# huangnengCSU/longcallR

Hardware: AMD Instinct MI355X
Metric: candidate_sites_per_sec (higher is better)
Workload: dtype u8 in, u32 counts, f64 likelihoods, i64 fixed-point phase scores

## Files before the change

### longcallr_amd/api.py

```python
import ctypes as C

import numpy as np

from . import _abi, _lib
from ._lib import LcrError


def _view(ptr, dtype, n):
    if n == 0 or not ptr:
        return np.zeros(0, dtype=dtype)
    buf = (C.c_char * (np.dtype(dtype).itemsize * n)).from_address(ptr)
    return np.frombuffer(buf, dtype=dtype, count=n).copy()


def _view_nocopy(ptr, dtype, n):
    if n == 0 or not ptr:
        return np.zeros(0, dtype=dtype)
    buf = (C.c_char * (np.dtype(dtype).itemsize * n)).from_address(ptr)
    return np.frombuffer(buf, dtype=dtype, count=n)


_DEBUG_ENV = {"LCR_PHASE_PROF": "phase_prof", "LCR_GRID_MIN_ENTRIES": "grid_min_entries",
              "LCR_GRID_GENERIC": "grid_generic", "LCR_GRID_SPEC_LANES": "grid_spec_lanes", "LCR_GRID_SPEC_BATCH": "grid_spec_batch", "LCR_POST_HALF": "post_half", "LCR_ENUM_FORCE_BIG": "enum_force_big",
              "LCR_ENUM_FORCE_STREAM": "enum_force_stream", "LCR_HIST_TILES": "hist_tiles", "LCR_TIE_ARITH": "tie_arith", "LCR_CHAIN_TIES": "chain_ties", "LCR_K3_HITS": "k3_hits", "LCR_FUSE_FILTER": "fuse_filter", "LCR_ASYNC_PHASE": "async_phase", "LCR_HOST_TRACE": "host_trace", "LCR_OWN_FILL": "own_fill", "LCR_REDO_LDS": "redo_lds", "LCR_SPEC_COMPACT": "spec_compact"}


class Engine:
    def __init__(self, device=0, params=None, timing=False):
        self.lib = _lib.load()
        h = C.c_void_p()
        rc = self.lib.lcr_ctx_create(device, C.byref(h))
        if rc != 0:
            raise LcrError("lcr_ctx_create(device=%d) failed with %d: no usable HIP device; "
                           "liblcr has no CPU fallback" % (device, rc))
        self.h = h
        self.device = device
        self.params = params if params is not None else _abi.make_params()
        self._sites = None
        self._keep = None
        self.last_truncated_columns = 0
        if timing:
            self.lib.lcr_enable_timing(self.h, 1)
            if timing is not True:
                self.debug_set("timing_mask", sum(1 << int(k) for k in timing))
        import os
        for env, key in _DEBUG_ENV.items():
            v = os.environ.get(env)
# ... 242 lines not shown
```

### longcallr_amd/csrc/k1_pileup.hip

```cpp
#include <algorithm>
#include <climits>

#include "lcr_dev.h"
#include "k2_eval.h"

#ifdef LCR_K1_ABLATE
#define K1_ABL LCR_K1_ABLATE
#else
#define K1_ABL 0
#endif
#ifndef K1_THREADS
#define K1_THREADS LCR_TILE
#endif
#define K1_WAVES (K1_THREADS / 64)
#define K1_CPT (LCR_TILE / K1_THREADS)
#define K1_RPB 2
#define K1_PMAP (8 * K1_THREADS)
#ifndef K1_NT_STORES
#define K1_NT_STORES 0
#endif
#ifndef K1_PIF
#define K1_PIF 4
#endif

// ... 165 lines not shown
  P_DIFF_DEPTH_R,
  P_DIFF_TS0,
  P_DIFF_TS1,
  P_DIFF_D,
  P_DIFF_N,
  P_NI,
  P_MM_F,
  P_MM_R = P_MM_F + 4,
  P_NPL = P_MM_R + 4
};
#define TSTRIDE (LCR_TILE + 1)
#define REF_PAD 16

__device__ __forceinline__ int block_incl_scan(int v, int* wsum ) {
  const int lane = threadIdx.x & 63, w = threadIdx.x >> 6;
  int s = wave_incl_scan(v);
  if (lane == 63) wsum[w] = s;
  __syncthreads();
  int add = 0;
  for (int i = 0; i < w; i++) add += wsum[i];
  return s + add;
}

__global__ void __launch_bounds__(K1_THREADS)
k1_pileup(BatchView b, DevParams prm, const int32_t* __restrict__ tile_region, const int32_t* __restrict__ tile_col0,
          int64_t n_cols, const int32_t* __restrict__ tile_fill, const int32_t* __restrict__ ent_off, const uint2* __restrict__ ents,
          const unsigned long long* __restrict__ recs,
          const int32_t* __restrict__ tile_nbase, uint32_t* __restrict__ planes, const int32_t* __restrict__ order,
          const int32_t* __restrict__ n_full, BinomTable bt, uint8_t* __restrict__ flt_flags, int32_t* __restrict__ flt_count) {
  if ((int)blockIdx.x >= *n_full) return;
  const int tile = order[blockIdx.x];
  __shared__ uint32_t pl[P_NPL * TSTRIDE];
  __shared__ __attribute__((aligned(16))) uint8_t refl[REF_PAD + LCR_TILE + 32];
  __shared__ unsigned long long rec_s[K1_RPB * K1_THREADS];
  __shared__ int pstart[K1_RPB * K1_THREADS + 1];
  __shared__ uint16_t pown[K1_PMAP];
  __shared__ int wsum[K1_WAVES];

  const int tid = threadIdx.x;
  const int g = tile_region[tile];
  const int tc0 = tile_col0[tile];
  const int vec = b.len[g];
  const int tlen = min(LCR_TILE, vec - tc0);
  const int64_t gcol0 = b.col_off[g] + tc0;
  if (*b.error_flag != 0) return;
  __shared__ uint32_t vge[17], vlt[17];
// ... 176 lines not shown
    __syncthreads();
  }

  const uint32_t nbase = (uint32_t)tile_nbase[tile];
  static_assert(K1_CPT == 1, "the fused filter counts one column per thread");
  int n_pass = 0;
  for (int col = tid; col < tlen; col += K1_THREADS) {
    const uint8_t R = refl[REF_PAD + col];
    const int ri = R == 'A' ? 0 : R == 'C' ? 1 : R == 'G' ? 2 : R == 'T' ? 3 : -1;
    uint32_t f[4], rv[4];
    uint32_t sf = 0, sr = 0;
#pragma unroll
    for (int k = 0; k < 4; k++) {
      const int hk = k < 2 ? k : 5 - k;
      f[k] = pl[(P_MM_F + hk) * TSTRIDE + col]; rv[k] = pl[(P_MM_R + hk) * TSTRIDE + col];
      sf += f[k]; sr += rv[k];
    }
    if (ri >= 0) {
      const uint32_t mf = pl[P_DIFF_DEPTH_F * TSTRIDE + col] - sf, mr = pl[P_DIFF_DEPTH_R * TSTRIDE + col] - sr;
#pragma unroll
      for (int k = 0; k < 4; k++) if (k == ri) { f[k] = mf; rv[k] = mr; }
    }
    const int64_t o = gcol0 + col;
#pragma unroll
    for (int k = 0; k < 4; k++) {
      planes[(int64_t)(LCR_PL_A + k) * n_cols + o] = f[k] + rv[k];
      planes[(int64_t)(LCR_PL_FWD_A + k) * n_cols + o] = f[k];
    }
    planes[(int64_t)LCR_PL_N * n_cols + o] = nbase + pl[P_DIFF_N * TSTRIDE + col];
    planes[(int64_t)LCR_PL_D * n_cols + o] = pl[P_DIFF_D * TSTRIDE + col];
    planes[(int64_t)LCR_PL_NI * n_cols + o] = pl[P_NI * TSTRIDE + col];
    planes[(int64_t)LCR_PL_TS_FWD * n_cols + o] = pl[P_DIFF_TS0 * TSTRIDE + col];
    planes[(int64_t)LCR_PL_TS_REV * n_cols + o] = pl[P_DIFF_TS1 * TSTRIDE + col];
    if (flt_flags) {
      uint32_t cnt[4];
#pragma unroll
      for (int k = 0; k < 4; k++) cnt[k] = f[k] + rv[k];
      const ColEval ev = eval_counts(cnt, R, prm, bt, [&]() { return pl[P_DIFF_D * TSTRIDE + col]; }, [&]() { return nbase + pl[P_DIFF_N * TSTRIDE + col]; },
                                     [&](int k) { return f[k]; });
      flt_flags[o] = ev.pass ? 1 : 0;
      n_pass += ev.pass ? 1 : 0;
    }
  }
  if (flt_flags) {
    const int total = __syncthreads_count(n_pass);
    if (tid == 0) flt_count[tile] = total;
  }
}

__global__ void __launch_bounds__(128) k1_empty_tiles(BatchView b, const int32_t* __restrict__ tile_region, const int32_t* __restrict__ tile_col0,
                                                       int64_t n_cols, const int32_t* __restrict__ tile_nbase, uint32_t* __restrict__ planes,
                                                       const int32_t* __restrict__ order, const int32_t* __restrict__ n_full, int n_tiles) {
  const int nf = *n_full;
  if (*b.error_flag != 0) return;
  const int bt = blockIdx.x, lt = threadIdx.x;
  if (bt + nf >= n_tiles) return;
  const int tile = order[nf + bt];
  const int g = tile_region[tile], tc0 = tile_col0[tile];
  const int tlen = min(LCR_TILE, b.len[g] - tc0);
  const int64_t gcol0 = b.col_off[g] + tc0;
  const uint32_t nb = (uint32_t)tile_nbase[tile];
  for (int col = lt * 4; col < tlen; col += 128 * 4) {
// ... 120 lines not shown
  for (int i = 0; i < w; i++) { run_d += ws[i][0]; run_c += ws[i][1]; }
  int e_before = ie - my_e;
  for (int i = 0; i < w; i++) e_before += we[i];
  if (tid < 33) hist[tid] = 0;
  __syncthreads();
#pragma unroll
  for (int x = 0; x < 4; x++) {
    const int t = t0 + x;
    if (t < n_tiles) {
      run_d += vd[x]; tile_nbase[t] = run_d;
      ent_off[t] = run_c; run_c += vc[x];
      if (cls[x] == 32) {
        order[base[32] + e_before++] = t;
        if (flt_count) flt_count[t] = 0;
      } else order[base[cls[x]] + atomicAdd(&hist[cls[x]], 1)] = t;
      if (t == n_tiles - 1) { ent_off[n_tiles] = run_c; tmp->n_full = n_tiles - tmp->cls_cnt[32]; }
    }
  }
}

void launch_k1_pileup(const BatchView& b, const DevParams& p, const int32_t* tile_region, const int32_t* tile_col0,
                      int32_t n_tiles, int64_t n_cols, const int32_t* tile_fill, const int32_t* ent_off, const void* ents,
                      const unsigned long long* recs, const int32_t* tile_nbase, uint32_t* planes, const int32_t* order ,
                      const int32_t* tiles_tmp, hipStream_t s, uint8_t* flt_flags, int32_t* flt_count) {
  static const BinomTable bt = make_binom_table();
  if (n_tiles == 0) return;
  hipLaunchKernelGGL(k1_pileup, dim3(n_tiles), dim3(K1_THREADS), 0, s, b, p, tile_region, tile_col0, n_cols, tile_fill, ent_off,
                     (const uint2*)ents, recs, tile_nbase, planes, order, tiles_tmp + 80 , bt, flt_flags, flt_count);
}
void launch_k1_empty_tiles(const BatchView& b, const int32_t* tile_region, const int32_t* tile_col0, int32_t n_tiles, int64_t n_cols,
                           const int32_t* tile_nbase, uint32_t* planes, const int32_t* order, const int32_t* tiles_tmp, hipStream_t s) {
  if (n_tiles == 0) return;
  hipLaunchKernelGGL(k1_empty_tiles, dim3(n_tiles), dim3(128), 0, s, b, tile_region, tile_col0, n_cols, tile_nbase, planes, order, tiles_tmp + 80, n_tiles);
}
size_t launch_k1_tiles_tmp_words(int32_t n_tiles) { return 88 + 2 * (size_t)((n_tiles + TS_TILES - 1) / TS_TILES) + 8; }
void launch_k1_tiles_a(int32_t n_tiles, const int32_t* tile_fill, const int32_t* tile_ndiff, const int32_t* tile_nent, int32_t* tmp ,
                       const unsigned int* acct, int32_t n_acct, K0Ctl* ctl, K0Ctl* host_ctl, const int32_t* tile_region,
                       const int32_t* tile_col0, const int32_t* region_len, hipStream_t s) {
  const int nb = (n_tiles + TS_TILES - 1) / TS_TILES;
  hipLaunchKernelGGL(k1_tiles_a, dim3(nb), dim3(256), 0, s, tile_fill, tile_ndiff, tile_nent, n_tiles, (TileScanTmp*)tmp, (int2*)(tmp + 88), acct, n_acct, ctl, host_ctl,
                     tile_region, tile_col0, region_len);
}
void launch_k1_tiles_b(int32_t n_tiles, const int32_t* tile_fill, const int32_t* tile_ndiff, const int32_t* tile_nent, int32_t* tmp,
                       int32_t* tile_nbase, int32_t* ent_off, int32_t* order, int32_t* flt_count, hipStream_t s) {
  const int nb = (n_tiles + TS_TILES - 1) / TS_TILES;
  hipLaunchKernelGGL(k1_tiles_b, dim3(nb), dim3(256), 0, s, tile_fill, tile_ndiff, tile_nent, n_tiles, (TileScanTmp*)tmp, (const int2*)(tmp + 88),
                     tile_nbase, ent_off, order, flt_count);
}

__global__ void __launch_bounds__(LCR_BLOCK)
k1_zonefix(BatchView b, int D, int L, int64_t n_cols, uint32_t* __restrict__ planes) {
// ... 234 lines not shown
```

### longcallr_amd/csrc/lcr_api.hip

```cpp
#include <chrono>
#include <cmath>
#include <cstdlib>
#include <map>
#include <mutex>

#include "lcr_ctx.h"

namespace {
struct BlockCache {
  std::mutex mu;
  std::multimap<size_t, void*> blocks[2][16];
  size_t held[2][16] = {};
  size_t limit[2] = {(size_t)24 << 30, (size_t)2 << 30};
};
BlockCache& block_cache() { static BlockCache* c = new BlockCache(); return *c; }
}
void* lcr_cache_take(int host, size_t want, size_t* cap) {
  int dev = 0;
  if (hipGetDevice(&dev) != hipSuccess || dev < 0 || dev >= 16) return nullptr;
  BlockCache& bc = block_cache();
  std::lock_guard<std::mutex> g(bc.mu);
  auto& m = bc.blocks[host ? 1 : 0][dev];
  auto it = m.lower_bound(want);
  if (it == m.end() || it->first > 2 * want + (1u << 20)) return nullptr;
// ... 440 lines not shown
        uint8_t* base = buf.as<uint8_t>();
        HIPCHK(c, lcr_fill_async(base + off, 0x5C, len, c->stream));
        std::fill(want.begin() + off, want.begin() + off + len, (uint8_t)0x5C);
        void* const ptrs[4] = {base + N + off, base + 2 * N + 3, nullptr, base + 3 * N + off};
        const int vals[4] = {0x80, 0, 7, 0xFF};
        const size_t sizes[4] = {len, 33, 0, len / 2};
        HIPCHK(c, lcr_fill_multi_async(4, ptrs, vals, sizes, c->stream));
        std::fill(want.begin() + N + off, want.begin() + N + off + len, (uint8_t)0x80);
        std::fill(want.begin() + 2 * N + 3, want.begin() + 2 * N + 3 + 33, (uint8_t)0);
        std::fill(want.begin() + 3 * N + off, want.begin() + 3 * N + off + len / 2, (uint8_t)0xFF);
        HIPCHK(c, hipMemcpyAsync(host.data(), buf.p, 4 * N, hipMemcpyDeviceToHost, c->stream));
        HIPCHK(c, hipStreamSynchronize(c->stream));
        if (host != want) { c->err = "fill_selftest: a fill kernel wrote other bytes than asked (offset " + std::to_string(off) + ", length " + std::to_string(len) + ")"; return LCR_E_DEVICE; }
      }
  }
  else if (k == "chain_ties") d.chain_ties = value != 0;
  else if (k == "redo_lds") d.redo_lds = (int)std::max<int64_t>(0, std::min<int64_t>(value, 128 * 1024));
  else if (k == "tie_arith") d.tie_arith = (int)std::max<int64_t>(0, std::min<int64_t>(value, 3));
  else if (k == "timing_mask") c->timing_mask = (uint32_t)value;
  else if (k == "hist_tiles") c->dbg_hist_tiles = value > 0 ? 1 : value < 0 ? -1 : 0;
  else if (k == "k3_hits") c->dbg_k3_hits = value != 0;
  else if (k == "fuse_filter") c->dbg_fuse_filter = value != 0;
  else if (k == "spec_compact") c->dbg_spec_compact = value != 0;
  else if (k == "poison_planes") c->dbg_poison_planes = value != 0;
  else if (k == "grid_spec_batch") d.spec_batch = (int)value;
  else if (k == "grid_spec_lanes") d.spec_lanes = (int)std::max<int64_t>(1, std::min<int64_t>(value, 16));
  else { c->err = "lcr_debug_set: unknown key " + k; return LCR_E_ARG; }
  return LCR_OK;
}

int lcr_get_ld_blocks(lcr_ctx* c, int32_t region, int32_t* n_blocks, const int32_t** block_off, const int32_t** snp_idx) {
  if (!c || !n_blocks || !block_off || !snp_idx) return LCR_E_ARG;
  if (c->stage < ST_PHASED) { c->err = "lcr_get_ld_blocks before lcr_phase"; return LCR_E_STATE; }
  if (region < 0 || region >= c->bv.n_regions) { c->err = "lcr_get_ld_blocks: no such region"; return LCR_E_ARG; }
  { int rc = phase_settle(c); if (rc) return rc; }
  PhaseInputs in;
  in.n_regions = c->bv.n_regions;
  in.cand_region_off = c->h_cand_off.data();
  const int rc = c->phase.ld_blocks(in, region, &c->ld_off, &c->ld_snps, c->stream, &c->err);
  if (rc != LCR_OK) return rc;
  *n_blocks = (int32_t)c->ld_off.size() - 1; *block_off = c->ld_off.data(); *snp_idx = c->ld_snps.data();
  return LCR_OK;
}

int lcr_get_tie_census(lcr_ctx* c, uint64_t out[8]) {
  if (!c || !out) return LCR_E_ARG;
// ... 8 lines not shown
```

### longcallr_amd/csrc/lcr_calls.hip

```cpp
#include "lcr_ctx.h"

int cand_settle(lcr_ctx* c) {
  if (!c->cand_pending) return LCR_OK;
  HIPCHK(c, hipEventSynchronize(c->ev_cand));
  const int ng = c->bv.n_regions;
  memcpy(c->h_cand_off.data(), c->h_stage[2].p, (size_t)(ng + 1) * 4);
  c->h_cand.assign(c->h_stage[1].as<lcr_candidate>(), c->h_stage[1].as<lcr_candidate>() + c->h_cand_off[ng]);
  c->cand_pending = false;
  return LCR_OK;
}

int frag_settle(lcr_ctx* c) {
  if (!c->nnz_pending) return LCR_OK;
  HIPCHK(c, hipEventSynchronize(c->ev_nnz));
  c->nnz = c->h_nnz.as<int64_t>()[c->bv.n_regions];
  c->nnz_pending = false;
  return LCR_OK;
}

namespace {

void cand_begin(lcr_ctx* c) {
  c->res_valid = false;
  rewind_to(c, ST_PILED);
// ... 13 lines not shown
  c->stage = ST_CALLED;
  return LCR_OK;
}

int cand_host_blocks(lcr_ctx* c, size_t n_max, lcr_candidate** hp, int32_t** ho) {
  const int ng = c->bv.n_regions;
  HIPCHK(c, c->h_stage[1].reserve(std::max<size_t>(n_max, 1) * sizeof(lcr_candidate)));
  HIPCHK(c, c->h_stage[2].reserve((size_t)(ng + 1) * 4));
  HIPCHK(c, c->h_stage[1].dev(hp));
  HIPCHK(c, c->h_stage[2].dev(ho));
  if (ng == 0) c->h_stage[2].as<int32_t>()[0] = 0;
  return LCR_OK;
}

int cand_queue_pass1(lcr_ctx* c) {
  const int nt = c->n_tiles;
  HIPCHK(c, c->flags.reserve(std::max<size_t>(c->n_cols, 1)));
  HIPCHK(c, c->tile_count.reserve(std::max(nt, 1) * 4));
  HIPCHK(c, c->tile_off.reserve((std::max(nt, 1) + 1) * 4));
  HIPCHK(c, c->total.reserve(16));
  const DevParams &fa = c->flt_dp, &fb = c->dp;
  const bool have_flt = c->flt_fused && c->dbg_fuse_filter != 0 && fa.ont == fb.ont && fa.min_depth == fb.min_depth && fa.max_depth == fb.max_depth && fa.low_cnt_cut == fb.low_cnt_cut &&
                        fa.use_strand_bias == fb.use_strand_bias && fa.min_af_intron == fb.min_af_intron && fa.low_frac_cut == fb.low_frac_cut && fa.sor_threshold == fb.sor_threshold;
  Timer t(c, LCR_K_CAND_FILTER);
  if (!have_flt) {
    c->flt_fused = false;
    launch_k2_filter(c->bv, c->dp, c->tile_region.as<int32_t>(), c->tile_col0.as<int32_t>(), nt, c->n_cols,
                     c->planes.as<uint32_t>(), c->k0_tile_fill.as<int32_t>(), c->flags.as<uint8_t>(), c->tile_count.as<int32_t>(), c->stream);
  }
  return LCR_OK;
}

void queue_compact(lcr_ctx* c, int32_t cap) {
  launch_k2_compact(c->bv, c->dp, c->tile_region.as<int32_t>(), c->tile_col0.as<int32_t>(), c->n_tiles, c->n_cols,
                    c->planes.as<uint32_t>(), c->flags.as<uint8_t>(), c->tile_count.as<int32_t>(), c->tile_off.as<int32_t>(),
                    c->survivors.as<Survivor>(), cap, c->stream);
}

int cand_count_survivors(lcr_ctx* c, int32_t* n_sv_out, bool* compacted) {
  const int ng = c->bv.n_regions, nt = c->n_tiles;
  HIPCHK(c, c->sv_region_off.reserve((ng + 1) * 4));
  HIPCHK(c, c->h_stage[0].reserve((ng + 2) * 4));
  int32_t* const sv_off = c->h_stage[0].as<int32_t>();
  { int32_t* d_sv = nullptr;
    HIPCHK(c, c->h_stage[0].dev(&d_sv));
    launch_scan_i32(c->scan_tmp, c->tile_count.as<int32_t>(), c->tile_off.as<int32_t>(), nt, c->total.as<int32_t>(), c->stream);
// ... 116 lines not shown
  const int64_t* d_pos = nullptr; const uint8_t* d_gt = nullptr; const float* d_q = nullptr;
  { int rc = upload(c, c->imp_pos, pos0, (size_t)n_sites, &d_pos, mem); if (rc) return rc; }
  { int rc = upload(c, c->imp_gt, genotype, (size_t)n_sites, &d_gt, mem); if (rc) return rc; }
  { int rc = upload(c, c->imp_q, qual, (size_t)n_sites, &d_q, mem); if (rc) return rc; }
  if (mem == LCR_MEM_DEVICE && n_sites > 0) {
    HIPCHK(c, c->h_imp_bad.reserve(64));
    int32_t* bad = c->h_imp_bad.as<int32_t>();
    *bad = 0;
    int32_t* d_bad = nullptr;
    HIPCHK(c, c->h_imp_bad.dev(&d_bad));
    launch_k2_import_check(d_pos, d_gt, n_sites, d_bad, c->stream);
    HIPCHK(c, hipEventRecord(c->ev_imp, c->stream));
    HIPCHK(c, hipEventSynchronize(c->ev_imp));
    if (*(volatile int32_t*)bad) { c->err = "lcr_import_candidates: sites must be sorted by position without duplicates, genotype codes 0-4"; return LCR_E_ARG; }
  }
  cand_begin(c);
  HIPCHK(c, c->imp_cnt.reserve(std::max(ng, 1) * 4));
  HIPCHK(c, c->d_cand.reserve(std::max<size_t>(n_sites, 1) * sizeof(lcr_candidate)));
  HIPCHK(c, c->d_cand_off.reserve((ng + 1) * 4));
  lcr_candidate* hp = nullptr; int32_t* ho = nullptr;
  { int rc = cand_host_blocks(c, (size_t)n_sites, &hp, &ho); if (rc) return rc; }
  c->h_cand.clear();
  c->h_cand_off.assign(ng + 1, 0);
  { Timer t(c, LCR_K_CAND_IMPORT);
    launch_k2_import_count(c->bv, d_pos, d_gt, d_q, n_sites, c->imp_cnt.as<int32_t>(), c->stream);
    launch_scan_i32(c->scan_tmp, c->imp_cnt.as<int32_t>(), c->d_cand_off.as<int32_t>(), ng, c->d_cand_off.as<int32_t>() + ng, c->stream);
    launch_k2_import_emit(c->bv, c->n_cols, c->planes.as<uint32_t>(), c->k0_tile_fill.as<int32_t>(), d_pos, d_gt, d_q, n_sites, c->d_cand_off.as<int32_t>(),
                          c->d_cand.as<lcr_candidate>(), c->stream, hp, ho); }
  const int rc = cand_tail(c);
  HT("import:ret");
  return rc;
}

int lcr_get_candidates(lcr_ctx* c, lcr_candidate_list* out) {
  if (!c || !out) return LCR_E_ARG;
  if (c->stage < ST_CALLED) { c->err = "lcr_get_candidates before lcr_candidates"; return LCR_E_STATE; }
  { int rc = cand_settle(c); if (rc) return rc; }
  { int rc = phase_settle(c); if (rc) return rc; }
  out->n_cand = (int32_t)c->h_cand.size();
  out->n_regions = c->bv.n_regions;
  out->cand = c->h_cand.data();
  out->region_off = c->h_cand_off.data();
  return LCR_OK;
}

int lcr_get_candidates_device(lcr_ctx* c, const lcr_candidate** dev_cand, int32_t* n_cand) {
// ... 111 lines not shown
```

### longcallr_amd/csrc/lcr_ctx.h

```cpp
#pragma once
#include <algorithm>
#include <cstring>

#include "lcr_dev.h"
#include "lcr_phase_host.h"

enum Stage { ST_NONE, ST_LOADED, ST_PILED, ST_CALLED, ST_FRAGGED, ST_PHASED };

struct lcr_ctx {
  int device = 0;
  hipStream_t stream = nullptr;
  bool own_stream = false;
  std::string err;
  Stage stage = ST_NONE;

  BatchView bv{};
  int64_t n_cols = 0, n_bases = 0, n_cigar = 0;
  int32_t n_tiles = 0;
  std::vector<int64_t> h_start0, h_col_off;
  std::vector<int32_t> h_len, h_read_begin, h_region_first_tile;
  DevBuf in_[16];
  struct UploadSlot { DevBuf buf[16]; hipEvent_t ev = nullptr; bool filled = false; lcr_reads rd{}; lcr_regions rg{}; } up[2];
  hipStream_t up_stream = nullptr;
  int bound_slot = -1;
  bool bound_host = false;
  DevBuf scan_tmp, read_region, read_bin, read_rend, tile_region, tile_col0, first_tile, k0_tile_fill, k0_items, tile_nbase, tile_order;
  DevBuf desc_tile, desc_val, chunks, chunk_off;
  DevBuf blk_first_read, read_scan, cig_compact, cig_off_new, cig_new_off32;
  uint64_t cig0 = 0;
  uint32_t n_ops = 0;
  int64_t n_items = 0;

  bool planes_dense = false;
  int dbg_poison_planes = 0;
  DevBuf planes;
  DevParams dp{};
  int32_t pile_platform = -1; uint32_t pile_dist_to_end = 0;
  float sor_thr = -1.f;
  HostBuf h_planes;
  HostBuf h_nnz;
  DevBuf region_e_off, frag_tmp_col, frag_tmp_val;
  hipEvent_t ev_ctl = nullptr, ev_sv = nullptr, ev_cand = nullptr, ev_nnz = nullptr, ev_imp = nullptr;
  int32_t sv_cap_guess = 0;
  bool nnz_pending = false, cand_pending = false;
  HostBuf h_order;
  static constexpr int UP_LANES = 4;
  HostBuf h_up[2 * UP_LANES]; hipEvent_t ev_up[2 * UP_LANES] = {}; bool up_busy[2 * UP_LANES] = {};
  HostBuf h_stage[4];

  bool cand_used = false;
  DevBuf flags, tile_count, tile_off, total, survivors, sv_region_off, hist, cand_tmp, keep;
  DevBuf hit_cnt, hit_list, ovf_list;
  bool hits_valid = false; int32_t hits_n_sv = 0;
  int dbg_hist_tiles = 0;
  int dbg_spec_compact = 1;
  int dbg_fuse_filter = 1;
// ... 22 lines not shown
  std::vector<uint8_t> ds_rows; bool ds_rows_set = false;

  bool junc_valid = false;
  int32_t junc_n = 0, junc_ng = 0;
  DevBuf j_part, j_npair, j_part_off, j_pair_off, j_tsz, j_tbl_off, j_rows, j_keys, j_tbl_key, j_tbl_cnt, j_flag, j_koff, j_ck, j_cc, j_cg, j_off, d_junc;
  HostBuf h_junc_ctl, h_junc, h_junc_off;
  hipEvent_t ev_junc = nullptr;

  DevBuf rd_start, rd_end, rd_diff, rd_ex, rd_cnt, rd_off, rd_s, rd_e, rd_max;
  std::vector<int64_t> rl_start0;
  std::vector<int32_t> rl_len;
  std::vector<uint32_t> rl_max;

  bool timing = false;
  uint32_t timing_mask = 0;
  hipEvent_t ev[LCR_NKERNELS][2] = {};
  bool ev_valid[LCR_NKERNELS] = {};
  int64_t pileup_bytes = 0, stage_bytes = 0;
};

inline void rewind_to(lcr_ctx* c, Stage to) {
  if (c->stage > to) c->stage = to;
  if (to < ST_PILED) {
    c->planes_dense = false;
    c->flt_fused = false;
  }
  if (to < ST_CALLED) {
    c->hits_valid = false;
    c->cand_used = false;
  }
  if (to < ST_FRAGGED) c->ds_rows_set = false;
  if (to < ST_PHASED) c->junc_valid = false;
}

struct Timer {
  lcr_ctx* c; int k;
  bool on() const { return c->timing && (c->timing_mask == 0 || ((c->timing_mask >> k) & 1u)); }
  Timer(lcr_ctx* c_, int k_) : c(c_), k(k_) { if (on()) { (void)hipEventRecord(c->ev[k][0], c->stream); } }
  ~Timer() { if (on()) { (void)hipEventRecord(c->ev[k][1], c->stream); c->ev_valid[k] = true; } }
};

inline DevParams to_dev(const lcr_params* p, float sor_thr) {
  DevParams d{};
  d.ont = p->platform == LCR_PLATFORM_ONT;
  d.dist_to_end = (int32_t)p->dist_to_end;
  d.polya_len = (int32_t)p->polya_len;
  d.min_baseq = p->min_baseq; d.min_depth = p->min_depth; d.max_depth = p->max_depth; d.min_qual = p->min_qual;
  d.low_cnt_cut = p->low_cnt_cut; d.min_linkers = p->min_linkers; d.use_strand_bias = p->use_strand_bias;
  d.min_af = p->min_af; d.min_af_intron = p->min_af_intron; d.low_frac_cut = p->low_frac_cut;
  d.sor_threshold = sor_thr;
  return d;
}

int upload_bytes(lcr_ctx* c, void* dst, const void* src, size_t bytes, hipStream_t q = nullptr);

template <class T>
int upload(lcr_ctx* c, DevBuf& buf, const T* src, size_t n, const T** dst, int mem) {
  if (mem == LCR_MEM_DEVICE) { *dst = src; return LCR_OK; }
  HIPCHK(c, buf.reserve(std::max<size_t>(n, 1) * sizeof(T)));
  if (n) { const int rc = upload_bytes(c, buf.p, src, n * sizeof(T)); if (rc) return rc; }
  *dst = buf.as<T>();
  return LCR_OK;
}

inline int phase_settle(lcr_ctx* c) { return c->phase.settle(&c->err); }
int cand_settle(lcr_ctx* c);
int frag_settle(lcr_ctx* c);
```

### longcallr_amd/csrc/lcr_dev.h

```cpp
#pragma once
#include <hip/hip_runtime.h>
#include <climits>
#include <cstddef>
#include <stdint.h>

#include <string>
#include <vector>

#include "../../include/lcr.h"

#ifndef LCR_TILE
#define LCR_TILE 256
#endif
#define LCR_BLOCK 256
#define LCR_WAVE 64

struct BatchView {
  int32_t n_reads, n_regions;
  int64_t n_bases;
  const int32_t* pos;
  const int32_t* seq_len;
  const int32_t* lead;
  const int32_t* trail;
  const uint8_t* flags;
// ... 161 lines not shown
  size_t nch;
  size_t cur;
  size_t acct;
  size_t tmp;
  size_t words;
};
inline PileScratch pile_scratch(int32_t n_tiles) {
  const size_t nt = (size_t)n_tiles;
  PileScratch L{};
  L.ctl = nt + 1; L.ndiff = nt + 16; L.nch = L.ndiff + nt + 8; L.cur = L.nch + nt + 8; L.acct = L.cur + nt + 8;
  L.tmp = L.acct + launch_k0_acct_words();
  L.words = (L.tmp + launch_k1_tiles_tmp_words(n_tiles) + 63) & ~(size_t)63;
  return L;
}
void launch_k1_tiles_a(int32_t n_tiles, const int32_t* tile_fill, const int32_t* tile_ndiff, const int32_t* tile_nent, int32_t* tmp ,
                       const unsigned int* acct, int32_t n_acct, K0Ctl* ctl, K0Ctl* host_ctl ,
                       const int32_t* tile_region, const int32_t* tile_col0, const int32_t* region_len , hipStream_t s);
void launch_k1_tiles_b(int32_t n_tiles, const int32_t* tile_fill, const int32_t* tile_ndiff, const int32_t* tile_nent, int32_t* tmp,
                       int32_t* tile_nbase, int32_t* ent_off, int32_t* order, int32_t* flt_count , hipStream_t s);
void launch_k1_pileup(const BatchView& b, const DevParams& p, const int32_t* tile_region, const int32_t* tile_col0,
                      int32_t n_tiles, int64_t n_cols, const int32_t* tile_fill, const int32_t* chunk_off, const void* chunks,
                      const unsigned long long* recs, const int32_t* tile_nbase, uint32_t* planes, const int32_t* order,
                      const int32_t* tiles_tmp , hipStream_t s,
                      uint8_t* flt_flags , int32_t* flt_count );
void launch_k1_empty_tiles(const BatchView& b, const int32_t* tile_region, const int32_t* tile_col0, int32_t n_tiles, int64_t n_cols,
                           const int32_t* tile_nbase, uint32_t* planes, const int32_t* order, const int32_t* tiles_tmp, hipStream_t s);
void launch_k1_zonefix(const BatchView& b, const ReadBin* rbin, int D, int L, int64_t n_cols, uint32_t* planes, hipStream_t s);
void launch_k2_filter(const BatchView& b, const DevParams& p, const int32_t* tile_region, const int32_t* tile_col0,
                      int32_t n_tiles, int64_t n_cols, const uint32_t* planes, const int32_t* tile_fill, uint8_t* flags,
                      int32_t* tile_count, hipStream_t s);
void launch_gather_i32(const int32_t* src, const int32_t* idx, int32_t n, int32_t n_src, const int32_t* total, int32_t* out, hipStream_t s,
                       int32_t* host_out = nullptr );
void launch_scan_i32(DevBuf& tmp, const int32_t* in, int32_t* out_excl, int32_t n, int32_t* total, hipStream_t s);
void launch_k2_compact(const BatchView& b, const DevParams& p, const int32_t* tile_region, const int32_t* tile_col0,
                       int32_t n_tiles, int64_t n_cols, const uint32_t* planes, const uint8_t* flags,
                       const int32_t* tile_count, const int32_t* tile_off, Survivor* out, int32_t out_cap, hipStream_t s);
float lcr_device_sor_threshold(hipStream_t s);
#define LCR_HITS 16
void launch_k2_hist(const BatchView& b, const DevParams& p, const ReadBin* rbin, const Survivor* sv, const int32_t* tile_off , int32_t n_tiles, int32_t n_sv,
                    uint32_t* hist , int32_t* hit_cnt , void* hit_list ,
                    int32_t* ovf_cnt , int32_t* ovf_list , hipStream_t s);
void launch_k2_hist_tiles(const BatchView& b, const int32_t* tile_col0, int32_t n_tiles, const int32_t* tile_count,
                          const int32_t* tile_off, const Survivor* sv, const int32_t* ent_off, const void* ents, const unsigned long long* recs,
                          uint32_t* hist, hipStream_t s);
void launch_k2_gt(const DevParams& p, const Survivor* sv, int32_t n_sv, const uint32_t* hist, const int64_t* start0,
                  lcr_candidate* out, int32_t* keep, hipStream_t s);
void launch_k2_finish(DevBuf& scan_tmp, const lcr_candidate* tmp, const int32_t* keep, int32_t n_sv, const int32_t* sv_region_off,
// ... 188 lines not shown
```

### longcallr_amd/csrc/lcr_pileup.hip

```cpp
#include "lcr_ctx.h"

namespace {

struct PilePools {
  int32_t n_blocks = 0;
  size_t pool_cap64 = 0, desc_cap64 = 0;
  size_t n_shards = 0;
  unsigned int pool_sub = 0, desc_sub = 0;
};

PilePools pile_size_pools(const lcr_ctx* c) {
  PilePools P;
  const int opb = launch_k0_opb();
  P.n_blocks = (int32_t)(((uint64_t)c->n_ops + opb - 1) / opb);
  P.desc_cap64 = (size_t)P.n_blocks * 128 + (size_t)c->bv.n_reads / 4 + 1024;
  P.pool_cap64 = (size_t)c->n_ops + (size_t)c->n_ops / 2 + (size_t)c->bv.n_reads + (size_t)c->n_bases / LCR_TILE + 8 * P.desc_cap64 + 1024;
  return P;
}

int pile_reserve_pools(lcr_ctx* c, PilePools& P) {
  const size_t nsh = P.n_shards = (size_t)launch_k0_acct_slots();
  const size_t pool_sub64 = (P.pool_cap64 + nsh - 1) / nsh + 256, desc_sub64 = (P.desc_cap64 + nsh - 1) / nsh + 64;
  if (pool_sub64 * nsh > 0xFFFFFFF0ull || desc_sub64 * nsh > 0x7FFFFFF0ull) { c->err = "batch too large for the 32-bit record pool: split it"; return LCR_E_ARG; }
  P.pool_sub = (unsigned int)pool_sub64; P.desc_sub = (unsigned int)desc_sub64;
// ... 7 lines not shown
int pile_reserve_scratch(lcr_ctx* c, const PileScratch& L) {
  const int nt = c->n_tiles;
  HIPCHK(c, c->k0_tile_fill.reserve(L.words * 4));
  c->bv.error_flag = &reinterpret_cast<K0Ctl*>(c->k0_tile_fill.as<int32_t>() + L.ctl)->error;
  HIPCHK(c, c->tile_order.reserve(std::max(nt, 1) * 4));
  HIPCHK(c, c->tile_nbase.reserve(std::max(nt, 1) * 4));
  HIPCHK(c, c->chunk_off.reserve(((size_t)nt + 2) * 4));
  HIPCHK(c, c->read_scan.reserve(std::max<size_t>(c->bv.n_reads, 1) * 8));
  HIPCHK(c, c->h_stage[0].reserve(64));
  return LCR_OK;
}

int pile_queue_k0(lcr_ctx* c, const PileScratch& L, const PilePools& P, bool& gated) {
  int32_t* const fill = c->k0_tile_fill.as<int32_t>();
  HIPCHK(c, lcr_fill_async(fill, 0, L.words * 4, c->stream));
  if (!gated) { HIPCHK(c, c->phase.gate_stream(c->stream)); gated = true; }
  Timer t(c, LCR_K_SPANS);
  launch_k0_ops(c->bv, c->read_bin.as<ReadBin>(), c->blk_first_read.as<int32_t>(), c->cig0, c->n_ops, c->dp.ont, c->dp.dist_to_end, c->n_tiles,
                fill, fill + L.nch, fill + L.ndiff, reinterpret_cast<K0Ctl*>(fill + L.ctl), (unsigned int*)(fill + L.acct), P.pool_sub, c->k0_items.as<unsigned long long>(),
                P.desc_sub, c->desc_tile.as<uint32_t>(), c->desc_val.p, c->read_scan.p, c->stream);
  return LCR_OK;
}

int pile_queue_tally(lcr_ctx* c, const PileScratch& L, const PilePools& P, bool fuse) {
  BatchView& b = c->bv;
  const int nt = c->n_tiles;
  int32_t* const fill = c->k0_tile_fill.as<int32_t>();
  K0Ctl* const d_ctl = reinterpret_cast<K0Ctl*>(fill + L.ctl);
  { Timer t(c, LCR_K_PILEUP);
    if (nt > 0) {
      K0Ctl* h_ctl_dev = nullptr;
      HIPCHK(c, c->h_stage[0].dev(&h_ctl_dev));
      launch_k1_tiles_a(nt, fill, fill + L.ndiff, fill + L.nch, fill + L.tmp, (unsigned int*)(fill + L.acct), launch_k0_acct_slots(),
                        d_ctl, h_ctl_dev, c->tile_region.as<int32_t>(), c->tile_col0.as<int32_t>(), b.len, c->stream);
    } else HIPCHK(c, hipMemcpyAsync(c->h_stage[0].p, d_ctl, sizeof(K0Ctl), hipMemcpyDeviceToHost, c->stream));
    HIPCHK(c, hipEventRecord(c->ev_ctl, c->stream));
    if (nt > 0) launch_k1_tiles_b(nt, fill, fill + L.ndiff, fill + L.nch, fill + L.tmp, c->tile_nbase.as<int32_t>(), c->chunk_off.as<int32_t>(),
                                  c->tile_order.as<int32_t>(), fuse ? c->tile_count.as<int32_t>() : nullptr, c->stream);
    if (nt > 0 && c->n_ops > 0)
      launch_k0_desc_bin(d_ctl, (const unsigned int*)(fill + L.acct), P.desc_sub, c->desc_tile.as<uint32_t>(), c->desc_val.p, c->chunk_off.as<int32_t>(), fill + L.cur,
                         c->chunks.p, P.n_blocks / 8 + 1, c->stream);
    launch_k1_pileup(b, c->dp, c->tile_region.as<int32_t>(), c->tile_col0.as<int32_t>(), nt, c->n_cols, fill, c->chunk_off.as<int32_t>(),
                     c->chunks.p, c->k0_items.as<unsigned long long>(), c->tile_nbase.as<int32_t>(), c->planes.as<uint32_t>(),
                     c->tile_order.as<int32_t>(), fill + L.tmp, c->stream, fuse ? c->flags.as<uint8_t>() : nullptr, fuse ? c->tile_count.as<int32_t>() : nullptr);
    if (!c->dp.ont && c->dp.dist_to_end > 0)
      launch_k1_zonefix(b, c->read_bin.as<ReadBin>(), c->dp.dist_to_end, c->dp.polya_len, c->n_cols, c->planes.as<uint32_t>(), c->stream); }
  HIPCHK(c, hipGetLastError());
  return LCR_OK;
}

int pile_read_verdict(lcr_ctx* c, K0Ctl* out, bool* retry) {
  HIPCHK(c, hipEventSynchronize(c->ev_ctl));
  HT("pile:ctl");
  *out = *c->h_stage[0].as<K0Ctl>();
  if (c->n_tiles == 0) out->empty_cols = 0;
  if (*c->h_order.as<int32_t>() != 0) { c->err = "the reads of a region must be sorted by position (lcr_reads.pos)"; return LCR_E_ARG; }
  if (out->error == 1) { c->err = "unknown CIGAR operation (reference panics: util.rs:944)"; return LCR_E_CIGAR; }
  if (out->error == 2) { c->err = "CIGAR inconsistent with l_seq / soft clips"; return LCR_E_CIGAR; }
  *retry = out->error != 0;
  return LCR_OK;
}

int planes_materialise(lcr_ctx* c) {
  if (c->planes_dense) return LCR_OK;
  launch_k1_empty_tiles(c->bv, c->tile_region.as<int32_t>(), c->tile_col0.as<int32_t>(), c->n_tiles, c->n_cols, c->tile_nbase.as<int32_t>(),
                        c->planes.as<uint32_t>(), c->tile_order.as<int32_t>(), c->k0_tile_fill.as<int32_t>() + pile_scratch(c->n_tiles).tmp, c->stream);
  HIPCHK(c, hipGetLastError());
  c->planes_dense = true;
  return LCR_OK;
}

}

extern "C" {

int lcr_pileup(lcr_ctx* c, const lcr_params* p) {
  HT("pileup");
  if (!c || !p) return LCR_E_ARG;
  if (c->stage < ST_LOADED) { c->err = "lcr_pileup before lcr_load_batch"; return LCR_E_STATE; }
  if (p->polya_len == 0) { c->err = "polya_len must be >= 1"; return LCR_E_ARG; }
  if ((uint64_t)c->bv.n_reads * 2ull * p->dist_to_end > 0x7FFFFF00ull * (uint64_t)LCR_BLOCK) { c->err = "dist_to_end x reads too large for one launch; split the batch"; return LCR_E_ARG; }
  HIPCHK(c, hipSetDevice(c->device));
  if (c->sor_thr < 0.f) c->sor_thr = lcr_device_sor_threshold(c->stream);
  c->dp = to_dev(p, c->sor_thr);
  c->dp.dbg = 0;
  HIPCHK(c, c->planes.reserve(std::max<size_t>((size_t)c->n_cols * LCR_NPLANES, 1) * 4));
  rewind_to(c, ST_LOADED);
  if (c->dbg_poison_planes) HIPCHK(c, lcr_fill_async(c->planes.p, 0xA5, (size_t)c->n_cols * LCR_NPLANES * 4, c->stream));
  const int nt = c->n_tiles;
  PilePools P = pile_size_pools(c);
  const PileScratch L = pile_scratch(nt);
  int rc;
  if ((rc = pile_reserve_scratch(c, L))) return rc;
  const bool fuse = c->dbg_fuse_filter != 0 && c->dp.ont && nt > 0;
  if (fuse) { HIPCHK(c, c->flags.reserve(std::max<size_t>(c->n_cols, 1))); HIPCHK(c, c->tile_count.reserve(std::max(nt, 1) * 4)); }
  K0Ctl ctl{};
  bool gated = false;
  for (bool retry = true; retry;) {
    if ((rc = pile_reserve_pools(c, P))) return rc;
    if ((rc = pile_queue_k0(c, L, P, gated))) return rc;
    if ((rc = pile_queue_tally(c, L, P, fuse))) return rc;
    if ((rc = pile_read_verdict(c, &ctl, &retry))) return rc;
    if (retry) {
      P.pool_cap64 = std::max<size_t>(P.pool_cap64 * 2, ((size_t)ctl.pool_top + 1024) * P.n_shards);
      P.desc_cap64 = std::max<size_t>(P.desc_cap64 * 2, ((size_t)ctl.desc_top + 1024) * P.n_shards);
    }
  }
  c->n_items = (int32_t)ctl.n_recs;
  const int64_t plane_cols = c->n_cols - (int64_t)ctl.empty_cols;
  c->pileup_bytes = c->n_bases + 8 * (int64_t)(int32_t)ctl.n_items + c->n_cols + 4 * LCR_NPLANES * plane_cols;
  c->stage_bytes = c->n_bases + 4 * c->n_cigar + 37 * (int64_t)c->bv.n_reads + c->n_cols + 4 * LCR_NPLANES * plane_cols;
  c->stage = ST_PILED;
  c->flt_fused = fuse; c->flt_dp = c->dp;
  c->pile_platform = p->platform; c->pile_dist_to_end = p->dist_to_end;
  return LCR_OK;
}

int lcr_get_columns(lcr_ctx* c, lcr_columns* out) {
  if (!c || !out) return LCR_E_ARG;
  if (c->stage < ST_PILED) { c->err = "lcr_get_columns before lcr_pileup"; return LCR_E_STATE; }
  HIPCHK(c, hipSetDevice(c->device));
  { int rc = planes_materialise(c); if (rc) return rc; }
  const size_t bytes = (size_t)c->n_cols * LCR_NPLANES * 4;
  HIPCHK(c, c->h_planes.reserve(std::max<size_t>(bytes, 1)));
  if (bytes) HIPCHK(c, hipMemcpyAsync(c->h_planes.p, c->planes.p, bytes, hipMemcpyDeviceToHost, c->stream));
  HIPCHK(c, hipStreamSynchronize(c->stream));
  out->n_cols = c->n_cols;
  out->planes = c->h_planes.as<uint32_t>();
  return LCR_OK;
}

}
```

Before: 6.291 billion.

## Store pileup planes only for filter-surviving columns, rematerialise lazily on demand

When the filter is fused into the pileup kernel, the kernel now writes the per-column count planes only for columns that pass the candidate filter, skipping the global stores for all other columns. A planes level state tracks how complete the planes are, and the full pileup kernel is rerun, followed by empty-tile fill, whenever a later stage or a host readback needs every column. This cuts memory write traffic on the common path. The cost is a second pileup pass when the fused filter cannot be reused or when plane data is imported.

```diff
diff --git a/longcallr_amd/api.py b/longcallr_amd/api.py
--- a/longcallr_amd/api.py
+++ b/longcallr_amd/api.py
@@ -22,7 +22,7 @@
 
 _DEBUG_ENV = {"LCR_PHASE_PROF": "phase_prof", "LCR_GRID_MIN_ENTRIES": "grid_min_entries",
               "LCR_GRID_GENERIC": "grid_generic", "LCR_GRID_SPEC_LANES": "grid_spec_lanes", "LCR_GRID_SPEC_BATCH": "grid_spec_batch", "LCR_POST_HALF": "post_half", "LCR_ENUM_FORCE_BIG": "enum_force_big",
-              "LCR_ENUM_FORCE_STREAM": "enum_force_stream", "LCR_HIST_TILES": "hist_tiles", "LCR_TIE_ARITH": "tie_arith", "LCR_CHAIN_TIES": "chain_ties", "LCR_K3_HITS": "k3_hits", "LCR_FUSE_FILTER": "fuse_filter", "LCR_ASYNC_PHASE": "async_phase", "LCR_HOST_TRACE": "host_trace", "LCR_OWN_FILL": "own_fill", "LCR_REDO_LDS": "redo_lds", "LCR_SPEC_COMPACT": "spec_compact"}
+              "LCR_ENUM_FORCE_STREAM": "enum_force_stream", "LCR_HIST_TILES": "hist_tiles", "LCR_TIE_ARITH": "tie_arith", "LCR_CHAIN_TIES": "chain_ties", "LCR_K3_HITS": "k3_hits", "LCR_FUSE_FILTER": "fuse_filter", "LCR_ASYNC_PHASE": "async_phase", "LCR_HOST_TRACE": "host_trace", "LCR_OWN_FILL": "own_fill", "LCR_REDO_LDS": "redo_lds", "LCR_SPEC_COMPACT": "spec_compact", "LCR_SURVIVOR_PLANES": "survivor_planes"}
 
 
 class Engine:
diff --git a/longcallr_amd/csrc/k1_pileup.hip b/longcallr_amd/csrc/k1_pileup.hip
--- a/longcallr_amd/csrc/k1_pileup.hip
+++ b/longcallr_amd/csrc/k1_pileup.hip
@@ -211,6 +211,7 @@
   return s + add;
 }
 
+template <bool SURVIVORS>
 __global__ void __launch_bounds__(K1_THREADS)
 k1_pileup(BatchView b, DevParams prm, const int32_t* __restrict__ tile_region, const int32_t* __restrict__ tile_col0,
           int64_t n_cols, const int32_t* __restrict__ tile_fill, const int32_t* __restrict__ ent_off, const uint2* __restrict__ ents,
@@ -433,22 +434,26 @@
       for (int k = 0; k < 4; k++) if (k == ri) { f[k] = mf; rv[k] = mr; }
     }
     const int64_t o = gcol0 + col;
-#pragma unroll
-    for (int k = 0; k < 4; k++) {
-      planes[(int64_t)(LCR_PL_A + k) * n_cols + o] = f[k] + rv[k];
-      planes[(int64_t)(LCR_PL_FWD_A + k) * n_cols + o] = f[k];
-    }
-    planes[(int64_t)LCR_PL_N * n_cols + o] = nbase + pl[P_DIFF_N * TSTRIDE + col];
-    planes[(int64_t)LCR_PL_D * n_cols + o] = pl[P_DIFF_D * TSTRIDE + col];
-    planes[(int64_t)LCR_PL_NI * n_cols + o] = pl[P_NI * TSTRIDE + col];
-    planes[(int64_t)LCR_PL_TS_FWD * n_cols + o] = pl[P_DIFF_TS0 * TSTRIDE + col];
-    planes[(int64_t)LCR_PL_TS_REV * n_cols + o] = pl[P_DIFF_TS1 * TSTRIDE + col];
+    auto store_planes = [&]() {
+#pragma unroll
+      for (int k = 0; k < 4; k++) {
+        planes[(int64_t)(LCR_PL_A + k) * n_cols + o] = f[k] + rv[k];
+        planes[(int64_t)(LCR_PL_FWD_A + k) * n_cols + o] = f[k];
+      }
+      planes[(int64_t)LCR_PL_N * n_cols + o] = nbase + pl[P_DIFF_N * TSTRIDE + col];
+      planes[(int64_t)LCR_PL_D * n_cols + o] = pl[P_DIFF_D * TSTRIDE + col];
+      planes[(int64_t)LCR_PL_NI * n_cols + o] = pl[P_NI * TSTRIDE + col];
+      planes[(int64_t)LCR_PL_TS_FWD * n_cols + o] = pl[P_DIFF_TS0 * TSTRIDE + col];
+      planes[(int64_t)LCR_PL_TS_REV * n_cols + o] = pl[P_DIFF_TS1 * TSTRIDE + col];
+    };
+    if (!SURVIVORS) store_planes();
     if (flt_flags) {
       uint32_t cnt[4];
 #pragma unroll
       for (int k = 0; k < 4; k++) cnt[k] = f[k] + rv[k];
       const ColEval ev = eval_counts(cnt, R, prm, bt, [&]() { return pl[P_DIFF_D * TSTRIDE + col]; }, [&]() { return nbase + pl[P_DIFF_N * TSTRIDE + col]; },
                                      [&](int k) { return f[k]; });
+      if (SURVIVORS && ev.pass) store_planes();
       flt_flags[o] = ev.pass ? 1 : 0;
       n_pass += ev.pass ? 1 : 0;
     }
@@ -615,11 +620,15 @@
 void launch_k1_pileup(const BatchView& b, const DevParams& p, const int32_t* tile_region, const int32_t* tile_col0,
                       int32_t n_tiles, int64_t n_cols, const int32_t* tile_fill, const int32_t* ent_off, const void* ents,
                       const unsigned long long* recs, const int32_t* tile_nbase, uint32_t* planes, const int32_t* order ,
-                      const int32_t* tiles_tmp, hipStream_t s, uint8_t* flt_flags, int32_t* flt_count) {
+                      const int32_t* tiles_tmp, hipStream_t s, uint8_t* flt_flags, int32_t* flt_count, bool survivors_only) {
   static const BinomTable bt = make_binom_table();
   if (n_tiles == 0) return;
-  hipLaunchKernelGGL(k1_pileup, dim3(n_tiles), dim3(K1_THREADS), 0, s, b, p, tile_region, tile_col0, n_cols, tile_fill, ent_off,
-                     (const uint2*)ents, recs, tile_nbase, planes, order, tiles_tmp + 80 , bt, flt_flags, flt_count);
+  if (survivors_only && flt_flags)
+    hipLaunchKernelGGL(k1_pileup<true>, dim3(n_tiles), dim3(K1_THREADS), 0, s, b, p, tile_region, tile_col0, n_cols, tile_fill, ent_off,
+                       (const uint2*)ents, recs, tile_nbase, planes, order, tiles_tmp + 80 , bt, flt_flags, flt_count);
+  else
+    hipLaunchKernelGGL(k1_pileup<false>, dim3(n_tiles), dim3(K1_THREADS), 0, s, b, p, tile_region, tile_col0, n_cols, tile_fill, ent_off,
+                       (const uint2*)ents, recs, tile_nbase, planes, order, tiles_tmp + 80 , bt, flt_flags, flt_count);
 }
 void launch_k1_empty_tiles(const BatchView& b, const int32_t* tile_region, const int32_t* tile_col0, int32_t n_tiles, int64_t n_cols,
                            const int32_t* tile_nbase, uint32_t* planes, const int32_t* order, const int32_t* tiles_tmp, hipStream_t s) {
diff --git a/longcallr_amd/csrc/lcr_api.hip b/longcallr_amd/csrc/lcr_api.hip
--- a/longcallr_amd/csrc/lcr_api.hip
+++ b/longcallr_amd/csrc/lcr_api.hip
@@ -486,6 +486,7 @@
   else if (k == "k3_hits") c->dbg_k3_hits = value != 0;
   else if (k == "fuse_filter") c->dbg_fuse_filter = value != 0;
   else if (k == "spec_compact") c->dbg_spec_compact = value != 0;
+  else if (k == "survivor_planes") c->dbg_survivor_planes = value != 0;
   else if (k == "poison_planes") c->dbg_poison_planes = value != 0;
   else if (k == "grid_spec_batch") d.spec_batch = (int)value;
   else if (k == "grid_spec_lanes") d.spec_lanes = (int)std::max<int64_t>(1, std::min<int64_t>(value, 16));
diff --git a/longcallr_amd/csrc/lcr_calls.hip b/longcallr_amd/csrc/lcr_calls.hip
--- a/longcallr_amd/csrc/lcr_calls.hip
+++ b/longcallr_amd/csrc/lcr_calls.hip
@@ -59,6 +59,7 @@
   const DevParams &fa = c->flt_dp, &fb = c->dp;
   const bool have_flt = c->flt_fused && c->dbg_fuse_filter != 0 && fa.ont == fb.ont && fa.min_depth == fb.min_depth && fa.max_depth == fb.max_depth && fa.low_cnt_cut == fb.low_cnt_cut &&
                         fa.use_strand_bias == fb.use_strand_bias && fa.min_af_intron == fb.min_af_intron && fa.low_frac_cut == fb.low_frac_cut && fa.sor_threshold == fb.sor_threshold;
+  if (!have_flt) { const int rc = planes_materialise(c, PL_RECORD_TILES); if (rc) return rc; }
   Timer t(c, LCR_K_CAND_FILTER);
   if (!have_flt) {
     c->flt_fused = false;
@@ -221,6 +222,7 @@
   { int rc = cand_host_blocks(c, (size_t)n_sites, &hp, &ho); if (rc) return rc; }
   c->h_cand.clear();
   c->h_cand_off.assign(ng + 1, 0);
+  { const int rc = planes_materialise(c, PL_RECORD_TILES); if (rc) return rc; }
   { Timer t(c, LCR_K_CAND_IMPORT);
     launch_k2_import_count(c->bv, d_pos, d_gt, d_q, n_sites, c->imp_cnt.as<int32_t>(), c->stream);
     launch_scan_i32(c->scan_tmp, c->imp_cnt.as<int32_t>(), c->d_cand_off.as<int32_t>(), ng, c->d_cand_off.as<int32_t>() + ng, c->stream);
diff --git a/longcallr_amd/csrc/lcr_ctx.h b/longcallr_amd/csrc/lcr_ctx.h
--- a/longcallr_amd/csrc/lcr_ctx.h
+++ b/longcallr_amd/csrc/lcr_ctx.h
@@ -6,6 +6,7 @@
 #include "lcr_phase_host.h"
 
 enum Stage { ST_NONE, ST_LOADED, ST_PILED, ST_CALLED, ST_FRAGGED, ST_PHASED };
+enum PlanesLevel { PL_SURVIVORS, PL_RECORD_TILES, PL_ALL };
 
 struct lcr_ctx {
   int device = 0;
@@ -31,7 +32,8 @@
   uint32_t n_ops = 0;
   int64_t n_items = 0;
 
-  bool planes_dense = false;
+  int planes_level = PL_SURVIVORS;
+  int dbg_survivor_planes = 1;
   int dbg_poison_planes = 0;
   DevBuf planes;
   DevParams dp{};
@@ -100,7 +102,7 @@
 inline void rewind_to(lcr_ctx* c, Stage to) {
   if (c->stage > to) c->stage = to;
   if (to < ST_PILED) {
-    c->planes_dense = false;
+    c->planes_level = PL_SURVIVORS;
     c->flt_fused = false;
   }
   if (to < ST_CALLED) {
@@ -142,5 +144,6 @@
 }
 
 inline int phase_settle(lcr_ctx* c) { return c->phase.settle(&c->err); }
+int planes_materialise(lcr_ctx* c, PlanesLevel level);
 int cand_settle(lcr_ctx* c);
 int frag_settle(lcr_ctx* c);
diff --git a/longcallr_amd/csrc/lcr_dev.h b/longcallr_amd/csrc/lcr_dev.h
--- a/longcallr_amd/csrc/lcr_dev.h
+++ b/longcallr_amd/csrc/lcr_dev.h
@@ -207,7 +207,8 @@
                       int32_t n_tiles, int64_t n_cols, const int32_t* tile_fill, const int32_t* chunk_off, const void* chunks,
                       const unsigned long long* recs, const int32_t* tile_nbase, uint32_t* planes, const int32_t* order,
                       const int32_t* tiles_tmp , hipStream_t s,
-                      uint8_t* flt_flags , int32_t* flt_count );
+                      uint8_t* flt_flags , int32_t* flt_count ,
+                      bool survivors_only );
 void launch_k1_empty_tiles(const BatchView& b, const int32_t* tile_region, const int32_t* tile_col0, int32_t n_tiles, int64_t n_cols,
                            const int32_t* tile_nbase, uint32_t* planes, const int32_t* order, const int32_t* tiles_tmp, hipStream_t s);
 void launch_k1_zonefix(const BatchView& b, const ReadBin* rbin, int D, int L, int64_t n_cols, uint32_t* planes, hipStream_t s);
diff --git a/longcallr_amd/csrc/lcr_pileup.hip b/longcallr_amd/csrc/lcr_pileup.hip
--- a/longcallr_amd/csrc/lcr_pileup.hip
+++ b/longcallr_amd/csrc/lcr_pileup.hip
@@ -53,7 +53,7 @@
   return LCR_OK;
 }
 
-int pile_queue_tally(lcr_ctx* c, const PileScratch& L, const PilePools& P, bool fuse) {
+int pile_queue_tally(lcr_ctx* c, const PileScratch& L, const PilePools& P, bool fuse, bool survivors_only) {
   BatchView& b = c->bv;
   const int nt = c->n_tiles;
   int32_t* const fill = c->k0_tile_fill.as<int32_t>();
@@ -73,7 +73,7 @@
                          c->chunks.p, P.n_blocks / 8 + 1, c->stream);
     launch_k1_pileup(b, c->dp, c->tile_region.as<int32_t>(), c->tile_col0.as<int32_t>(), nt, c->n_cols, fill, c->chunk_off.as<int32_t>(),
                      c->chunks.p, c->k0_items.as<unsigned long long>(), c->tile_nbase.as<int32_t>(), c->planes.as<uint32_t>(),
-                     c->tile_order.as<int32_t>(), fill + L.tmp, c->stream, fuse ? c->flags.as<uint8_t>() : nullptr, fuse ? c->tile_count.as<int32_t>() : nullptr);
+                     c->tile_order.as<int32_t>(), fill + L.tmp, c->stream, fuse ? c->flags.as<uint8_t>() : nullptr, fuse ? c->tile_count.as<int32_t>() : nullptr, survivors_only);
     if (!c->dp.ont && c->dp.dist_to_end > 0)
       launch_k1_zonefix(b, c->read_bin.as<ReadBin>(), c->dp.dist_to_end, c->dp.polya_len, c->n_cols, c->planes.as<uint32_t>(), c->stream); }
   HIPCHK(c, hipGetLastError());
@@ -92,15 +92,26 @@
   return LCR_OK;
 }
 
-int planes_materialise(lcr_ctx* c) {
-  if (c->planes_dense) return LCR_OK;
-  launch_k1_empty_tiles(c->bv, c->tile_region.as<int32_t>(), c->tile_col0.as<int32_t>(), c->n_tiles, c->n_cols, c->tile_nbase.as<int32_t>(),
-                        c->planes.as<uint32_t>(), c->tile_order.as<int32_t>(), c->k0_tile_fill.as<int32_t>() + pile_scratch(c->n_tiles).tmp, c->stream);
-  HIPCHK(c, hipGetLastError());
-  c->planes_dense = true;
-  return LCR_OK;
 }
 
+int planes_materialise(lcr_ctx* c, PlanesLevel level) {
+  const int nt = c->n_tiles;
+  int32_t* const fill = c->k0_tile_fill.as<int32_t>();
+  const PileScratch L = pile_scratch(nt);
+  if (c->planes_level < PL_RECORD_TILES && level >= PL_RECORD_TILES) {
+    launch_k1_pileup(c->bv, c->flt_dp, c->tile_region.as<int32_t>(), c->tile_col0.as<int32_t>(), nt, c->n_cols, fill, c->chunk_off.as<int32_t>(),
+                     c->chunks.p, c->k0_items.as<unsigned long long>(), c->tile_nbase.as<int32_t>(), c->planes.as<uint32_t>(),
+                     c->tile_order.as<int32_t>(), fill + L.tmp, c->stream, nullptr, nullptr, false);
+    HIPCHK(c, hipGetLastError());
+    c->planes_level = PL_RECORD_TILES;
+  }
+  if (c->planes_level < PL_ALL && level >= PL_ALL) {
+    launch_k1_empty_tiles(c->bv, c->tile_region.as<int32_t>(), c->tile_col0.as<int32_t>(), nt, c->n_cols, c->tile_nbase.as<int32_t>(),
+                          c->planes.as<uint32_t>(), c->tile_order.as<int32_t>(), fill + L.tmp, c->stream);
+    HIPCHK(c, hipGetLastError());
+    c->planes_level = PL_ALL;
+  }
+  return LCR_OK;
 }
 
 extern "C" {
@@ -124,13 +135,14 @@
   int rc;
   if ((rc = pile_reserve_scratch(c, L))) return rc;
   const bool fuse = c->dbg_fuse_filter != 0 && c->dp.ont && nt > 0;
+  const bool survivors_only = fuse && c->dbg_survivor_planes != 0;
   if (fuse) { HIPCHK(c, c->flags.reserve(std::max<size_t>(c->n_cols, 1))); HIPCHK(c, c->tile_count.reserve(std::max(nt, 1) * 4)); }
   K0Ctl ctl{};
   bool gated = false;
   for (bool retry = true; retry;) {
     if ((rc = pile_reserve_pools(c, P))) return rc;
     if ((rc = pile_queue_k0(c, L, P, gated))) return rc;
-    if ((rc = pile_queue_tally(c, L, P, fuse))) return rc;
+    if ((rc = pile_queue_tally(c, L, P, fuse, survivors_only))) return rc;
     if ((rc = pile_read_verdict(c, &ctl, &retry))) return rc;
     if (retry) {
       P.pool_cap64 = std::max<size_t>(P.pool_cap64 * 2, ((size_t)ctl.pool_top + 1024) * P.n_shards);
@@ -143,6 +155,7 @@
   c->stage_bytes = c->n_bases + 4 * c->n_cigar + 37 * (int64_t)c->bv.n_reads + c->n_cols + 4 * LCR_NPLANES * plane_cols;
   c->stage = ST_PILED;
   c->flt_fused = fuse; c->flt_dp = c->dp;
+  c->planes_level = survivors_only ? PL_SURVIVORS : PL_RECORD_TILES;
   c->pile_platform = p->platform; c->pile_dist_to_end = p->dist_to_end;
   return LCR_OK;
 }
@@ -151,7 +164,7 @@
   if (!c || !out) return LCR_E_ARG;
   if (c->stage < ST_PILED) { c->err = "lcr_get_columns before lcr_pileup"; return LCR_E_STATE; }
   HIPCHK(c, hipSetDevice(c->device));
-  { int rc = planes_materialise(c); if (rc) return rc; }
+  { int rc = planes_materialise(c, PL_ALL); if (rc) return rc; }
   const size_t bytes = (size_t)c->n_cols * LCR_NPLANES * 4;
   HIPCHK(c, c->h_planes.reserve(std::max<size_t>(bytes, 1)));
   if (bytes) HIPCHK(c, hipMemcpyAsync(c->h_planes.p, c->planes.p, bytes, hipMemcpyDeviceToHost, c->stream));
```

New measurement: 6.356 billion, median of 6. 1.0% higher.
